# citibeth/spsparse

Hardware: AMD Instinct MI355X
Metric: nnz(C)/s for C=A*A SpGEMM (higher is better)
Workload: dtype f64

## Files before the change

### spsparse_amd/build.py

```python
import os
import subprocess
import sys
from concurrent.futures import ThreadPoolExecutor

HERE = os.path.dirname(os.path.abspath(__file__))
CSRC = os.path.join(HERE, "csrc")
VARIANT = os.environ.get("SPSAMD_VARIANT", "")
LIBDIR = os.path.join(HERE, "lib", VARIANT) if VARIANT else os.path.join(HERE, "lib")
LIB = os.path.join(LIBDIR, "libspsparse_amd.so")
SOURCES = ["prims.hip", "operand.hip", "sink.hip", "consolidate.hip", "spgemm.hip", "symbolic_heavy.hip", "k_light.hip", "k_hash.hip", "k_dense.hip", "k_tiles.hip", "k_spmm.hip", "k_add.hip", "k_stream.hip", "k_masked.hip", "k_sampled.hip", "k_select.hip", "k_extract.hip", "k_reduce.hip", "k_emult.hip",
           "workload.hip", "capi.hip", "dist.hip"]
HEADERS = ["internal.h", "devutil.h", "spgemm_dev.h", "spgemm_host.h", "spgemm_hash.h", "workload_common.h", "x86fp.h", os.path.join("..", "..", "include", "spsparse_amd.h")]
FLAGS = ["--offload-arch=gfx950", "-O3", "-std=c++17", "-fPIC", "-ffp-contract=off",
         "-munsafe-fp-atomics", "-Wall", "-Wno-unused-result"]
FLAGS += os.environ.get("SPSAMD_CXXFLAGS", "").split()


def hipcc():
    for cand in (os.environ.get("HIPCC"), "/opt/rocm/bin/hipcc", "hipcc"):
        if cand and (os.path.isabs(cand) and os.path.exists(cand) or not os.path.isabs(cand)):
            return cand
    return "hipcc"


def _stale(target, deps):
    if not os.path.exists(target):
        return True
    t = os.path.getmtime(target)
    return any(os.path.getmtime(d) > t for d in deps)


def build(force=False, verbose=False):
    os.makedirs(LIBDIR, exist_ok=True)
    hdrs = [os.path.join(CSRC, h) for h in HEADERS]
    objs, jobs = [], []
    for s in SOURCES:
        src = os.path.join(CSRC, s)
        obj = os.path.join(LIBDIR, s.replace(".hip", ".o"))
        objs.append(obj)
        if force or _stale(obj, [src] + hdrs):
            jobs.append([hipcc()] + FLAGS + ["-c", src, "-o", obj])

    def run(cmd):
        if verbose:
            print(" ".join(cmd), flush=True)
        subprocess.check_call(cmd)

    with ThreadPoolExecutor(max_workers=6) as ex:
        list(ex.map(run, jobs))
    if force or jobs or _stale(LIB, objs):
        run([hipcc(), "--offload-arch=gfx950", "-shared", "-fPIC", "-o", LIB] + objs + ["-ldl"])
    return LIB


if __name__ == "__main__":
    print(build(force="--force" in sys.argv, verbose=True))
```

### spsparse_amd/csrc/k_dense.hip

```cpp
#include "spgemm_host.h"

namespace spsamd {


template <int W, int NT, int MODE, bool PAT>
__global__ __launch_bounds__(NT, 4) void k_dense(const Cell *cells, uint32_t ncell, const uint32_t *xb, RowMeta m,
	const uint32_t *widx, uint64_t kstride, uint64_t wstride, uint32_t narrow, EmitParams ep, SinkParams sk, uint32_t *claim_ctr)
{
	constexpr int NW = NT / 64;
	constexpr int NGRP = W / 64;
	constexpr int GPW = NGRP / NW;
	constexpr uint32_t WSHIFT = W == 8192 ? 13 : 14;
	constexpr int R = DENSE_R;
	constexpr int NWORD = W / 64;
	constexpr int WPL = NWORD / 64;
	__shared__ double acc[MODE == MODE_COUNT ? 1 : W + 64];
	__shared__ __attribute__((aligned(16))) uint8_t ctouch[MODE == MODE_COUNT ? W : 16];
	__shared__ uint32_t s_cpref[NT + 1];
	__shared__ uint2 s_cse[NT];
	__shared__ double s_caval[NT];
	__shared__ unsigned long long s_bmask[NWORD];
	__shared__ uint32_t s_scrL[2][NW], s_scrN[2][NW];
	__shared__ uint32_t s_wcnt[NW + 1];
	__shared__ PatCell s_pat;
	__shared__ unsigned long long s_u64[2 * NW];
	__shared__ double s_f64[NW];
	__shared__ uint32_t s_claim[4];

	const unsigned tid = threadIdx.x, lane = lane_id();
	const unsigned wv = (unsigned)__builtin_amdgcn_readfirstlane((int)wave_id());
	const double CLEAN = (PAT && MODE != MODE_COUNT) ? -0.0 : 0.0;
	if (MODE == MODE_COUNT) { for (int q = tid; q < W / 16; q += NT) reinterpret_cast<uint4 *>(ctouch)[q] = make_uint4(0, 0, 0, 0); }
	else for (int q = tid; q < W + 64; q += NT) acc[q] = CLEAN;
	for (int q = tid; q < NWORD; q += NT) s_bmask[q] = 0ull;
	const bool plain = ep.C == 1.0 && !ep.si_pos && !ep.sk_pos;
	const unsigned long long laneK = (unsigned long long)lane * 0x9E3779B97F4A7C15ull;
	unsigned long long d_cnt = 0, d_hash = 0; double d_sum = 0;
	PatAcc pat; pat_init(pat);
	if (tid == 0) pat_reset(&s_pat);
	uint32_t flip = 0;
#ifdef SPSAMD_STAMPS
	unsigned long long st_[12] = {}; unsigned long long st_t = clock64();
#endif

	constexpr uint32_t NONE = 0xFFFFFFFFu;
	const bool claimed = claim_ctr != nullptr && xb != nullptr && !ABL(ep, 16);
	const CellWalk walk = cell_walk(claimed ? nullptr : xb, ncell);
	const uint32_t stride = walk.stride, cend = walk.end;
	const uint32_t clast = ncell ? ncell - 1 : 0;
	uint32_t part = blockIdx.x & 7u, tried = 0;
	auto claim_resolve = [&](uint32_t got) -> uint32_t {
		while (true) {
			if (got < xb[part + 1]) return got;
// ... 66 lines not shown
		STAMP_COUNT(8);
		uint32_t pnseg = 0;
		for (uint32_t chunk = beg; chunk < end; chunk += NT) {
			STAMP_COUNT(9);
			uint32_t lo2, hi2; double a2;
			{
				seg_bounds(kA, w, lo2, hi2);
				a2 = aA;
				if (chunk + NT + tid >= end) hi2 = lo2;
				const uint32_t e2 = chunk + 2 * NT + tid;
				const uint32_t e2c = e2 < end ? e2 : beg;
				kA = m.acol[e2c]; aA = m.aval[e2c];
			}
			const uint32_t items = (len + R - 1) / R;
			const uint32_t inc = wave_inclusive_scan_u32(items);
			const uint64_t nzm = __ballot(len != 0);
			const uint32_t wrank = (uint32_t)__popcll(nzm & lanemask_lt());
			if (lane == 63) s_scrL[flip][wv] = inc;
			if (lane == 0) s_scrN[flip][wv] = (uint32_t)__popcll(nzm);
			STAMP(0);
			lds_barrier();
			STAMP(1);
			if (claimed && chunk == beg) {
				i2 = (uint32_t)__builtin_amdgcn_readfirstlane((int)s_claim[2 + (iter & 1u)]);
				pend2 = cell_pend_load(cells, min(i2, clast), zlane);
			}
			uint32_t baseL = 0, baseN = 0, total = 0, nzc = 0;
#pragma unroll
			for (int q = 0; q < NW; ++q) {
				const uint32_t l = s_scrL[flip][q], n = s_scrN[flip][q];
				if (q < (int)wv) { baseL += l; baseN += n; }
				total += l; nzc += n;
			}
			flip ^= 1u;
			total = (uint32_t)__builtin_amdgcn_readfirstlane((int)total);
			nzc = (uint32_t)__builtin_amdgcn_readfirstlane((int)nzc);
			const uint32_t myfirst = baseL + inc - items;
			if (len) {
				const uint32_t rank = baseN + wrank;
				s_cpref[rank] = myfirst;
				s_cse[rank] = make_uint2(lo, lo + len);
				s_caval[rank] = a;
				if (myfirst < (uint32_t)W) atomicOr(reinterpret_cast<uint32_t *>(s_bmask) + (myfirst >> 5), 1u << (myfirst & 31u));
			}
			if (ABL(ep, 8)) total = 0;
			if (total == 0) { lo = lo2; len = hi2 - lo2; a = a2; continue; }
			if (ep.ordered && MODE != MODE_COUNT) {
				lds_barrier();
				for (uint32_t q = 0; q < nzc; ++q) {
					const uint2 se = s_cse[q];
					const double aq = s_caval[q];
					for (uint32_t t = se.x + tid; t < se.y; t += NT) {
						const BTup bt = m.btup[t];
						const uint32_t slot = (uint32_t)bt.col - wbase;
						acc[slot] = acc[slot] + aq * btup_val(bt);
					}
					lds_barrier();
				}
				for (int q = tid; q < NWORD; q += NT) s_bmask[q] = 0ull;
				lo = lo2; len = hi2 - lo2; a = a2;
				continue;
			}
			uint32_t Q0 = 0;
			for (uint32_t pb = 0; pb < total; pb += W) {
				const uint32_t pe = min(total, pb + (uint32_t)W);
				if (pb) {
					lds_barrier();
					for (int q = tid; q < NWORD; q += NT) s_bmask[q] = 0ull;
					lds_barrier();
					if (len && myfirst >= pb && myfirst < pe) atomicOr(&s_bmask[(myfirst - pb) >> 6], 1ull << ((myfirst - pb) & 63u));
				}
				STAMP(2);
				lds_barrier();
				STAMP(3);
				unsigned long long mw[WPL]; uint32_t pre[WPL];
				uint32_t run = Q0;
#pragma unroll
				for (int x = 0; x < WPL; ++x) {
					mw[x] = s_bmask[x * 64 + lane];
					const uint32_t cnt = (uint32_t)__popcll(mw[x]);
					const uint32_t incl = wave_inclusive_scan_u32(cnt);
					pre[x] = run + incl - cnt;
					run += (uint32_t)__builtin_amdgcn_readlane((int)incl, 63);
				}
				const uint32_t nsteps = (pe - pb + NT - 1) / NT;
				auto lookup = [&](uint32_t step, uint32_t &obp, uint32_t &onv, double &oav) {
					const uint32_t b = step * NW + wv;
					const uint32_t t = pb + (b << 6) + lane;
					const bool ok = t < pe;
					uint32_t mlo = 0, mhi = 0, pr = 0;
#pragma unroll
					for (int x = 0; x < WPL; ++x) {
						if ((b >> 6) == (uint32_t)x) {
							mlo = (uint32_t)__builtin_amdgcn_readlane((int)(uint32_t)mw[x], (int)(b & 63u));
							mhi = (uint32_t)__builtin_amdgcn_readlane((int)(uint32_t)(mw[x] >> 32), (int)(b & 63u));
							pr = (uint32_t)__builtin_amdgcn_readlane((int)pre[x], (int)(b & 63u));
						}
					}
					if (ABL(ep, 128)) { obp = (t * R) & 0xFFFFFu; onv = ok ? R : 0u; oav = 1.0; return; }
					const uint32_t s1lo = (mlo >> 1) | (mhi << 31), s1hi = mhi >> 1;
					const uint32_t qs = pr + (mlo & 1u) - 1u;
					uint32_t q = qs + __builtin_amdgcn_mbcnt_hi(s1hi, __builtin_amdgcn_mbcnt_lo(s1lo, 0u));
					q = min(q, nzc - 1u);
					const uint2 se = s_cse[q];
					obp = se.x + (t - s_cpref[q]) * R;
					onv = ok ? min((uint32_t)R, se.y - obp) : 0u;
					oav = s_caval[q];
				};
				const char *bbase = reinterpret_cast<const char *>(m.btup);
				auto fetch = [&](uint32_t bp_) -> BPiece {
					if (ABL(ep, 64)) bp_ &= 0xFFFFu;
					if (narrow) return *reinterpret_cast<const BPiece *>(bbase + (uint32_t)((bp_ << 3) + (bp_ << 2)));
					return *reinterpret_cast<const BPiece *>(bbase + (uint64_t)bp_ * 12u);
				};
				auto accumulate = [&](const BPiece &piece, uint32_t nv_, double av_) {
#pragma unroll
					for (int u = 0; u < R; ++u) {
						const uint32_t slot = (uint32_t)u < nv_ ? (ABL(ep, 64) ? (piece.w[3 * u] & (W - 1)) : piece.w[3 * u] - wbase) : (uint32_t)W + lane;
						if (ABL(ep, 32)) { if (piece.w[3 * u + 2] == 0x7FF12345u) acc[MODE == MODE_COUNT ? 0 : slot] = av_; }
						else if (MODE == MODE_COUNT) { if ((uint32_t)u < nv_) ctouch[slot] = (uint8_t)1; }
						else {
							const double pv = av_ * __hiloint2double((int)piece.w[3 * u + 2], (int)piece.w[3 * u + 1]);
							atomicAdd(&acc[slot], pv);
							if (PAT && (uint32_t)u < nv_) pat_note(pat, pv);
						}
					}
				};
				STAMP(4);
#if DENSE_DEPTH == 2
				uint32_t bp0, nv0, bp1 = 0, nv1 = 0; double av0, av1 = 0.0;
				lookup(0, bp0, nv0, av0);
				BPiece p0 = fetch(bp0), p1 = p0;
				if (nsteps > 1) lookup(1, bp1, nv1, av1);
				for (uint32_t step = 0; step < nsteps; ++step) {
					STAMP_COUNT(10);
					if (step + 1 < nsteps) p1 = fetch(bp1);
					uint32_t bp2 = 0, nv2 = 0; double av2 = 0.0;
					if (step + 2 < nsteps) lookup(step + 2, bp2, nv2, av2);
					accumulate(p0, nv0, av0);
					p0 = p1; nv0 = nv1; av0 = av1;
					bp1 = bp2; nv1 = nv2; av1 = av2;
				}
#else
				uint32_t bp, nv; double av;
				lookup(0, bp, nv, av);
				for (uint32_t step = 0; step < nsteps; ++step) {
					STAMP_COUNT(10);
					const BPiece piece = fetch(bp);
					uint32_t nbp = bp, nnv = 0; double nav = 0.0;
					if (step + 1 < nsteps) lookup(step + 1, nbp, nnv, nav);
					accumulate(piece, nv, av);
					bp = nbp; nv = nnv; av = nav;
				}
#endif
				Q0 = run;
				STAMP(5);
			}
			if (PAT) { pat_publish(pat, &s_pat); pnseg += nzc; }
			lds_barrier();
			STAMP(6);
			for (int q = tid; q < NWORD; q += NT) s_bmask[q] = 0ull;
			lo = lo2; len = hi2 - lo2; a = a2;
		}
		{
			uint32_t l2, h2;
			seg_bounds(nk, rec1.wa, l2, h2);
			nlo = l2; nlen = nact ? h2 - l2 : 0u;
		}
		if (ABL(ep, 16)) continue;
		STAMP(0);
		uint32_t claim_pending = NONE;
		if (claimed && tid == 0 && tried < 8u) claim_pending = atomicAdd(&claim_ctr[part * 32u], 1u);
		const double pthr = PAT ? pat_threshold(&s_pat, pnseg) : -1.0;
		const uint32_t pbeg = beg, pend = end;
		double v[GPW];
		uint64_t nzmask[GPW];
		uint32_t wcount = 0;
		constexpr unsigned long long MIXK = 0x9E3779B97F4A7C15ull;
		unsigned long long X0 = ((((unsigned long long)(uint32_t)rowid) << 32) | (unsigned long long)(wbase + wv * GPW * 64u)) * MIXK;
		X0 = ((unsigned long long)(uint32_t)__builtin_amdgcn_readfirstlane((int)(uint32_t)(X0 >> 32)) << 32) |
			(unsigned long long)(uint32_t)__builtin_amdgcn_readfirstlane((int)(uint32_t)X0);
		double r_sum = 0;
		unsigned long long r_hash = 0;
		if constexpr (MODE == MODE_COUNT) {
			static_assert(W / 16 == NT, "sixteen flag bytes per thread");
			uint32_t cnt = 0;
			{
				uint4 *cw = reinterpret_cast<uint4 *>(ctouch);
				const uint4 x = cw[tid];
				const uint32_t xs[4] = {x.x, x.y, x.z, x.w};
				if (x.x | x.y | x.z | x.w) {
					cw[tid] = make_uint4(0, 0, 0, 0);
#pragma unroll
					for (int q = 0; q < 4; ++q) {
						if (!ep.sk_pos) cnt += (uint32_t)__popc(xs[q]);
						else {
#pragma unroll
							for (int b = 0; b < 4; ++b)
								if (((xs[q] >> (8 * b)) & 1u) && col_allowed(ep, (int32_t)(wbase + tid * 16u + (uint32_t)(4 * q + b)))) ++cnt;
						}
					}
				}
			}
			wcount = (uint32_t)wave_reduce_sum((unsigned long long)cnt);
		} else {
#pragma unroll
		for (int gi = 0; gi < GPW; ++gi) {
			int grp = wv * GPW + gi;
			double x = acc[grp * 64 + lane];
			acc[grp * 64 + lane] = CLEAN;
			bool ok;
			if (MODE != MODE_COUNT && PAT) {
				const bool touched = __double_as_longlong(x) != (long long)0x8000000000000000ull;
				x = pat_fix_wave(touched && !(fabs(x) > pthr), x, (int32_t)(wbase + grp * 64 + lane), m, pbeg, pend);
			}
			if (plain) ok = x != 0;
			else ok = emit_value(ep, a_scale, (int32_t)(wbase + grp * 64 + lane), x, &x);
			v[gi] = x;
			nzmask[gi] = __ballot(ok);
			wcount += (uint32_t)__popcll(nzmask[gi]);
			if (MODE == MODE_DIGEST) {
				unsigned long long h = X0 + laneK;
				h ^= h >> 29;
				r_hash += ok ? h : 0ull;
				if (plain && !PAT) r_sum += x;
				else r_sum += ok ? x : 0.0;
				X0 += 64ull * MIXK;
			}
		}
		}
		if (MODE == MODE_DIGEST) {
			if (lane == 0) d_cnt += wcount;
			d_sum += r_sum;
			d_hash += r_hash;
			if (sk.row_nnz) {
				double rs = wave_reduce_sum(r_sum);
				r_hash = wave_reduce_sum(r_hash);
				if (lane == 0 && wcount) { atomicAdd((unsigned long long *)&sk.row_nnz[rowid], (unsigned long long)wcount); atomicAdd(&sk.row_sum[rowid], rs); atomicAdd(&sk.row_hash[rowid], r_hash); }
			}
		} else {
			if (lane == 0) s_wcnt[wv] = wcount;
			__syncthreads();
			uint32_t wbefore = 0, wtotal = 0;
#pragma unroll
			for (int q = 0; q < NW; ++q) { uint32_t t = s_wcnt[q]; if (q < (int)wv) wbefore += t; wtotal += t; }
			if (MODE == MODE_COUNT) {
				if (tid == 0) sk.segcount[cell.seg] = wtotal;
			} else {
				int64_t o = sk.segoff[cell.seg] + wbefore;
#pragma unroll
				for (int gi = 0; gi < GPW; ++gi) {
					uint64_t mk = nzmask[gi];
					if ((mk >> lane) & 1ull) {
						int64_t oo = o + __popcll(mk & lanemask_lt());
						sk.out_i[oo] = rowid;
						sk.out_j[oo] = (int32_t)(wbase + (wv * GPW + gi) * 64 + lane);
						sk.out_v[oo] = v[gi];
					}
					o += __popcll(mk);
				}
				if (tid == 0) sk.segactual[cell.seg] = wtotal;
			}
			__syncthreads();
// ... 69 lines not shown
```

### spsparse_amd/csrc/k_tiles.hip

```cpp
#include "spgemm_host.h"
#include "spgemm_hash.h"

namespace spsamd {

constexpr uint32_t TILE_NONE = 0xFFFFFFFFu;


template <int MODE, bool PAT>
__global__ __launch_bounds__(TILE2_NT, 4) void k_hash_tiles2(const Tile *tiles, uint32_t ntile, const TCell *tcells, RowMeta m,
	const uint32_t *bwin, uint32_t nwin1, uint32_t narrow, EmitParams ep, SinkParams sk, uint32_t *claim_ctr)
{
	constexpr int NT = TILE2_NT, T = TILE2_T, NW = NT / 64, R = DENSE_R;
	constexpr int NWORD = TILE2_ITEMS / 64;
	constexpr int MAXST = 3;
	__shared__ int32_t h_key[T + 64];
	__shared__ double h_val[MODE == MODE_COUNT ? 1 : T];
	__shared__ uint16_t occ[T / 2];
	__shared__ uint64_t s_sort[MODE == MODE_STORE ? T / 2 : 1];
	__shared__ uint16_t s_cnt[MODE == MODE_STORE ? 16 * ((T / 2 + NT - 1) / NT) * (NT / 64) : 1];
	__shared__ TileX<NT, NWORD> X;
	__shared__ uint32_t scr32[NW + 1];
	__shared__ uint32_t s_nocc;
	__shared__ PatCell s_pat;
	__shared__ unsigned long long s_u64[2 * NW];
	__shared__ double s_f64[NW];
	__shared__ uint32_t s_claim[4];

	const unsigned tid = threadIdx.x, lane = lane_id();
	const unsigned wv = (unsigned)__builtin_amdgcn_readfirstlane((int)wave_id());
	for (int q = tid; q < T; q += NT) { h_key[q] = -1; if (MODE != MODE_COUNT) h_val[q] = 0.0; }
	if (tid < 64) h_key[T + tid] = -1;
	for (int q = tid; q < NWORD; q += NT) X.bmask[q] = 0ull;
	if (tid == 0) s_nocc = 0;
	PatAcc pat; pat_init(pat);
	if (tid == 0) pat_reset(&s_pat);
	DigestAcc dacc{0, 0, 0.0};
	uint32_t flip = 0;
	const char *bbase = reinterpret_cast<const char *>(m.btup);
#ifdef SPSAMD_STAMPS
	unsigned long long st_[12] = {}; unsigned long long st_t = clock64();
#endif

	const bool claimed = claim_ctr != nullptr;
	const uint32_t stride = gridDim.x;
	const uint32_t tlast = ntile - 1;
	uint32_t i0, i1;
	if (claimed) {
		if (tid == 0) for (int q = 0; q < 3; ++q) { const uint32_t got = atomicAdd(claim_ctr, 1u); s_claim[q == 2 ? 3 : q] = got < ntile ? got : TILE_NONE; }
		__syncthreads();
		i0 = s_claim[0]; i1 = s_claim[1];
	} else {
		i0 = blockIdx.x;
		i1 = i0 + stride < ntile ? i0 + stride : TILE_NONE;
	}
// ... 100 lines not shown
							const double pv = av * __hiloint2double((int)piece.w[3 * u + 2], (int)piece.w[3 * u + 1]);
							atomicAdd(&h_val[h[u]], pv);
							if (PAT) pat_note(pat, pv);
						}
					}
					newmask[u] = __ballot(isnew[u]);
					nnew += (uint32_t)__popcll(newmask[u]);
				}
				if (nnew) {
					uint32_t base = 0;
					if (lane == 0) base = lds_add_rtn_u32(&s_nocc, nnew);
					base = (uint32_t)__builtin_amdgcn_readfirstlane((int)base);
#pragma unroll
					for (int u = 0; u < R; ++u) {
						if (isnew[u]) occ[base + __popcll(newmask[u] & lanemask_lt())] = (uint16_t)h[u];
						base += (uint32_t)__popcll(newmask[u]);
					}
				}
			}
			if (PAT) pat_publish(pat, &s_pat);
			STAMP(3);
			lds_barrier();
			STAMP(4);
			const uint32_t nocc = s_nocc;
			if (c + 1 < tile.ncells) {
				tile_lookup(X, tab, nzc, (i1 >> 6) + wv, X.cellI[c + 2], pbp, pnv, pav);
				ppiece = fetch_piece(bbase, pbp, narrow);
			}
			uint32_t colbase = 0, colbits = 0;
			if (MODE == MODE_STORE) {
				const uint32_t wab = X.cellw[c];
				const uint32_t wa = wab & 0xFFFFu, wb = wab >> 16;
				colbase = wa << ep.wshift;
				colbits = ep.wshift + (wb - wa > 1 ? 32 - __builtin_clz(wb - wa - 1u) : 0);
			}
			STAMP(5);
			const double pthr = PAT ? pat_threshold(&s_pat, tile.end - tile.beg) : -1.0;
			hash_emit<T, NT, MODE, PAT>(nocc, rowid, seg, ep, sk, h_key, h_val, occ, s_sort, scr32, dacc, s_cnt, colbase, colbits, m, tile.beg, tile.end, pthr);
			if (PAT) { lds_barrier(); if (tid == 0) pat_reset(&s_pat); }
			if (tid == 0) s_nocc = 0;
			STAMP(6);
			lds_barrier();
			STAMP(7);
		}
		for (int q = tid; q < NWORD; q += NT) X.bmask[q] = 0ull;
	}
#ifdef SPSAMD_STAMPS
	if (tid == 0 && sk.stamps) for (int i = 0; i < 12; ++i) sk.stamps[(size_t)blockIdx.x * 12 + i] = st_[i];
#endif
	if (MODE == MODE_DIGEST) digest_flush<NT>(sk.digest, dacc.cnt, dacc.hash, dacc.sum, s_u64, s_f64);
}


template <int MODE, bool PAT>
__global__ __launch_bounds__(BM_NT, 4) void k_bm_tiles(const Tile *tiles, uint32_t ntile, const TCell *tcells, RowMeta m,
	const uint32_t *bwin, uint32_t nwin1, uint32_t narrow, EmitParams ep, SinkParams sk, uint32_t *claim_ctr)
{
	constexpr int NT = BM_NT, NW = NT / 64, R = DENSE_R;
	constexpr int NWORD = BM_ITEMS / 64;
	constexpr int MAXST = (BM_MAXOUT / R + (int)TILE_LMAX + 64 + NT - 1) / NT;
	constexpr int WPT = BM_WORDS / NT;
	__shared__ __attribute__((aligned(16))) unsigned long long bm[BM_WORDS];
	__shared__ __attribute__((aligned(8))) uint16_t bpre[BM_WORDS];
	__shared__ double acc[BM_MAXOUT];
	__shared__ uint32_t colof[BM_MAXOUT];
	__shared__ TileX<NT, NWORD> X;
	__shared__ uint32_t s_wtot[2][NW];
	__shared__ uint32_t s_wbase[NW];
	__shared__ PatCell s_pat;
	__shared__ uint32_t s_scan[NW + 1];
	__shared__ unsigned long long s_u64[2 * NW];
	__shared__ double s_f64[NW];
	__shared__ uint32_t s_claim[4];

	const unsigned tid = threadIdx.x, lane = lane_id();
	const unsigned wv = (unsigned)__builtin_amdgcn_readfirstlane((int)wave_id());
	for (int q = tid; q < BM_WORDS; q += NT) bm[q] = 0ull;
	for (int q = tid; q < BM_MAXOUT; q += NT) acc[q] = 0.0;
	for (int q = tid; q < NWORD; q += NT) X.bmask[q] = 0ull;
	const bool plain = ep.C == 1.0 && !ep.si_pos && !ep.sk_pos;
	unsigned long long d_cnt = 0, d_hash = 0; double d_sum = 0;
	PatAcc pat; pat_init(pat);
	if (PAT && tid == 0) pat_reset(&s_pat);
	uint32_t flip = 0, sflip = 0;
	const char *bbase = reinterpret_cast<const char *>(m.btup);
#ifdef SPSAMD_STAMPS
	unsigned long long st_[12] = {}; unsigned long long st_t = clock64();
#endif

	const bool claimed = claim_ctr != nullptr;
	const uint32_t stride = gridDim.x;
	const uint32_t tlast = ntile - 1;
	uint32_t i0, i1;
	if (claimed) {
		if (tid == 0) for (int q = 0; q < 3; ++q) { const uint32_t got = atomicAdd(claim_ctr, 1u); s_claim[q == 2 ? 3 : q] = got < ntile ? got : TILE_NONE; }
		__syncthreads();
		i0 = s_claim[0]; i1 = s_claim[1];
	} else {
		i0 = blockIdx.x;
		i1 = i0 + stride < ntile ? i0 + stride : TILE_NONE;
	}
	i0 = (uint32_t)__builtin_amdgcn_readfirstlane((int)i0); i1 = (uint32_t)__builtin_amdgcn_readfirstlane((int)i1);
	Tile rec1 = tiles[min(i0, tlast)];
	uint32_t nlo, nlen, nseg_, nw_; double na;
	{
		const uint32_t L = rec1.end - rec1.beg;
		uint32_t lsh = 0;
		while ((1u << lsh) < L) ++lsh;
		const uint32_t c = tid >> lsh, ei = tid & ((1u << lsh) - 1u);
		const bool act = c < rec1.ncells && ei < L;
		const uint32_t ec = rec1.beg + (ei < L ? ei : 0u);
		const TCell tc = tcells[rec1.first + (c < rec1.ncells ? c : 0u)];
		const uint32_t *bw = bwin + (uint64_t)(uint32_t)m.acol[ec] * nwin1;
		const uint32_t lo = bw[tc.wa], hi = bw[tc.wb];
// ... 36 lines not shown
		{
			const uint32_t *bw = bwin + (uint64_t)(uint32_t)nk * nwin1;
			const uint32_t nlo_ = bw[ntc.wa], nhi_ = bw[ntc.wb];
			nlo = nlo_; nlen = nact ? nhi_ - nlo_ : 0u; nseg_ = ntc.seg; nw_ = (uint32_t)ntc.wa | ((uint32_t)ntc.wb << 16);
		}
		if (total == 0 || nzc == 0) {
			if (MODE != MODE_DIGEST) for (uint32_t c = tid; c < tile.ncells; c += NT) { if (MODE == MODE_COUNT) sk.segcount[X.cellseg[c]] = 0; else sk.segactual[X.cellseg[c]] = 0; }
			continue;
		}
		TileTab<NWORD / 64> tab;
		tile_tables(X, tab);

		uint32_t pbp, pnv; double pav;
		tile_lookup(X, tab, nzc, (X.cellI[0] >> 6) + wv, X.cellI[1], pbp, pnv, pav);
		BPiece ppiece = fetch_piece(bbase, pbp, narrow);
#ifndef BM_D2
#define BM_D2 1
#endif
		constexpr bool D2 = BM_D2 && MODE != MODE_STORE;
		uint32_t qnv = 0; double qav = 0; BPiece qpiece;
		if (D2 && ((X.cellI[1] - X.cellI[0]) >> 6) > (uint32_t)NW + wv) {
			uint32_t qbp;
			tile_lookup(X, tab, nzc, (X.cellI[0] >> 6) + NW + wv, X.cellI[1], qbp, qnv, qav);
			qpiece = fetch_piece(bbase, qbp, narrow);
		}
		STAMP(0);
		for (uint32_t c = 0; c < tile.ncells; ++c) {
			STAMP_COUNT(11);
			const uint32_t i0 = X.cellI[c], i1 = X.cellI[c + 1];
			const uint32_t seg = X.cellseg[c];
			const uint32_t nblk = (i1 - i0) >> 6;
			const uint32_t wab = X.cellw[c];
			const uint32_t colbase = (wab & 0xFFFFu) << ep.wshift;
			const uint32_t nwords = ((wab >> 16) - (wab & 0xFFFFu)) << (ep.wshift - 6);
			if ((nblk > (uint32_t)(MAXST * NW) || nwords > (uint32_t)BM_WORDS) && tid == 0) atomicOr(sk.err, 2u);
			uint32_t krel[MAXST][R]; double kval[MODE == MODE_COUNT ? 1 : MAXST][MODE == MODE_COUNT ? 1 : R];
#pragma unroll
			for (int st = 0; st < MAXST; ++st) {
#pragma unroll
				for (int u = 0; u < R; ++u) krel[st][u] = 0xFFFFFFFFu;
				const uint32_t bl = (uint32_t)st * NW + wv;
				if (st > 0 && bl >= nblk) continue;
				uint32_t nv; double av; BPiece piece;
				if (st == 0) { nv = bl < nblk ? pnv : 0u; av = pav; piece = ppiece; }
				else if (D2 && st == 1) { nv = qnv; av = qav; piece = qpiece; }
				else {
					uint32_t bp;
					tile_lookup(X, tab, nzc, (i0 >> 6) + bl, i1, bp, nv, av);
					piece = fetch_piece(bbase, bp, narrow);
				}
#pragma unroll
				for (int u = 0; u < R; ++u) {
					if ((uint32_t)u < nv) {
						const uint32_t rel = piece.w[3 * u] - colbase;
						krel[st][u] = rel;
						if constexpr (MODE != MODE_COUNT) {
							kval[st][u] = av * __hiloint2double((int)piece.w[3 * u + 2], (int)piece.w[3 * u + 1]);
							if (PAT) pat_note(pat, kval[st][u]);
						}
						atomicOr(reinterpret_cast<uint32_t *>(bm) + (rel >> 5), 1u << (rel & 31u));
					}
				}
			}
			if (PAT && MODE != MODE_COUNT) pat_publish(pat, &s_pat);
			STAMP(2);
			lds_barrier();
			STAMP(3);
			const double pthr = (PAT && MODE != MODE_COUNT) ? pat_threshold(&s_pat, tile.end - tile.beg) : -1.0;
			uint32_t wcnt[WPT], mine = 0;
			{
				unsigned long long wd[WPT];
#pragma unroll
				for (int x = 0; x < WPT; ++x) wd[x] = bm[tid * WPT + x];
				if (c + 1 < tile.ncells) {
					const uint32_t i2 = X.cellI[c + 2];
					tile_lookup(X, tab, nzc, (i1 >> 6) + wv, i2, pbp, pnv, pav);
					ppiece = fetch_piece(bbase, pbp, narrow);
					if (D2 && ((i2 - i1) >> 6) > (uint32_t)NW + wv) {
						uint32_t qbp;
						tile_lookup(X, tab, nzc, (i1 >> 6) + NW + wv, i2, qbp, qnv, qav);
						qpiece = fetch_piece(bbase, qbp, narrow);
					}
				}
#pragma unroll
				for (int x = 0; x < WPT; ++x) { wcnt[x] = (uint32_t)__popcll(wd[x]); mine += wcnt[x]; }
			}
			const uint32_t inc = wave_inclusive_scan_u32(mine);
			if (lane == 63) s_wtot[sflip][wv] = inc;
			{
				static_assert(WPT == 4, "packed prefix store");
				const uint32_t r0 = inc - mine, r1 = r0 + wcnt[0], r2 = r1 + wcnt[1], r3 = r2 + wcnt[2];
				reinterpret_cast<uint2 *>(bpre)[tid] = make_uint2(r0 | (r1 << 16), r2 | (r3 << 16));
			}
			STAMP(4);
			lds_barrier();
			STAMP(5);
			if (PAT && MODE != MODE_COUNT && tid == 0) pat_reset(&s_pat);
			uint32_t distinct;
			{
				const uint32_t t = lane < (unsigned)NW ? s_wtot[sflip][lane] : 0u;
				const uint32_t ti = wave_inclusive_scan_u32(t);
				if (lane < (unsigned)NW) s_wbase[lane] = ti - t;
				distinct = (uint32_t)__builtin_amdgcn_readlane((int)ti, NW - 1);
			}
			sflip ^= 1u;
			if (MODE == MODE_COUNT && !ep.sk_pos) {
				if (tid == 0) sk.segcount[seg] = distinct;
#pragma unroll
				for (int x = 0; x < WPT; ++x) { const uint32_t w = tid * WPT + x; if (w < nwords && wcnt[x]) bm[w] = 0ull; }
				lds_barrier();
				continue;
			}
			STAMP(4);
			if constexpr (MODE != MODE_COUNT) {
#pragma unroll
				for (int st = 0; st < MAXST; ++st) {
					if ((uint32_t)st * NW + wv >= nblk) continue;
					uint32_t pre[R], wb[R]; unsigned long long wd[R];
#pragma unroll
					for (int u = 0; u < R; ++u) {
						const uint32_t w = (krel[st][u] >> 6) & (uint32_t)(BM_WORDS - 1);
						pre[u] = bpre[w]; wb[u] = s_wbase[w / (64 * WPT)]; wd[u] = bm[w];
					}
#pragma unroll
					for (int u = 0; u < R; ++u) {
						const uint32_t rel = krel[st][u];
						if (rel != 0xFFFFFFFFu) {
							const uint32_t rank = wb[u] + pre[u] + (uint32_t)__popcll(wd[u] & ((1ull << (rel & 63u)) - 1ull));
							atomicAdd(&acc[rank], kval[st][u]);
							colof[rank] = rel;
						}
					}
				}
				STAMP(6);
				lds_barrier();
				STAMP(7);
			}
			if constexpr (MODE != MODE_COUNT) {
				if (mine) { uint4 *z = reinterpret_cast<uint4 *>(&bm[tid * WPT]); z[0] = make_uint4(0, 0, 0, 0); z[1] = make_uint4(0, 0, 0, 0); }
			}
			if constexpr (MODE == MODE_DIGEST) {
				unsigned long long cnt = 0, rh = 0; double vs = 0;
				auto note = [&](uint32_t rel, double v) {
					const int32_t col = (int32_t)(colbase + rel);
					const bool ok = plain ? v != 0 : emit_value(ep, a_scale, col, v, &v);
					if (ok) { ++cnt; rh += mix64((uint32_t)rowid, (uint32_t)col); vs += v; }
				};
				if constexpr (!PAT) {
					unsigned long long *acc64 = reinterpret_cast<unsigned long long *>(acc);
					for (uint32_t i = tid; i < distinct; i += 2 * NT) {
						const uint32_t j = i + NT;
						const bool two = j < distinct;
						const uint32_t jj = two ? j : i;
						const uint32_t rel0 = colof[i], rel1 = colof[jj];
						const double v0 = __longlong_as_double((long long)atomicExch(&acc64[i], 0ull));
						const double v1 = __longlong_as_double((long long)atomicExch(&acc64[jj], 0ull));
						note(rel0, v0);
						if (two) note(rel1, v1);
					}
				} else {
					for (uint32_t base = 0; base < distinct; base += NT) {
						const uint32_t i = base + tid;
						const bool valid = i < distinct;
						const uint32_t rel = valid ? colof[i] : 0u;
						double v = valid ? acc[i] : 0.0;
						if (valid) acc[i] = 0.0;
						v = pat_fix_wave(valid && !(fabs(v) > pthr), v, (int32_t)(colbase + rel), m, tile.beg, tile.end);
						if (valid) note(rel, v);
					}
				}
				d_cnt += cnt; d_sum += vs; d_hash += rh;
				if (sk.row_nnz) {
					const unsigned long long rc = wave_reduce_sum(cnt); const double rs = wave_reduce_sum(vs);
					rh = wave_reduce_sum(rh);
					if (lane == 0 && rc) { atomicAdd((unsigned long long *)&sk.row_nnz[rowid], rc); atomicAdd(&sk.row_sum[rowid], rs); atomicAdd(&sk.row_hash[rowid], rh); }
				}
			} else if constexpr (MODE == MODE_COUNT) {
				uint32_t cnt = 0;
#pragma unroll
				for (int x = 0; x < WPT; ++x) {
					if (!wcnt[x]) continue;
					const uint32_t w = tid * WPT + x;
					unsigned long long word = bm[w];
					bm[w] = 0ull;
					while (word) {
						const uint32_t bit = (uint32_t)__builtin_ctzll(word);
						word &= word - 1ull;
						if (col_allowed(ep, (int32_t)(colbase + (w << 6) + bit))) ++cnt;
					}
				}
				uint32_t tot;
				block_exclusive_scan<uint32_t, NT>(cnt, s_scan, &tot);
				if (tid == 0) sk.segcount[seg] = tot;
			} else {
				const int64_t o = sk.segoff[seg];
				uint32_t nbad = 0, run = 0;
				int any_bad;
				if (!ep.sk_pos) {
					for (uint32_t base = 0; base < distinct; base += NT) {
						const uint32_t i = base + tid;
						const bool valid = i < distinct;
						const uint32_t rel = valid ? colof[i] : 0u;
						double v = 1.0;
						if (valid) { v = acc[i]; acc[i] = 0.0; }
						if (PAT) v = pat_fix_wave(valid && !(fabs(v) > pthr), v, (int32_t)(colbase + rel), m, tile.beg, tile.end);
						const bool ok = !valid || (plain ? v != 0 : emit_value(ep, a_scale, (int32_t)(colbase + rel), v, &v));
						if (valid) { sk.out_i[o + i] = rowid; sk.out_j[o + i] = ok ? (int32_t)(colbase + rel) : -1; sk.out_v[o + i] = v; }
						if (!ok) ++nbad;
					}
					any_bad = __syncthreads_or((int)nbad);
					if (any_bad) {
						for (uint32_t ibase = 0; ibase < distinct; ibase += NT) {
							const uint32_t i = ibase + tid;
							int32_t col = -1; double v = 0;
							if (i < distinct) { col = sk.out_j[o + i]; v = sk.out_v[o + i]; }
							const bool ok = col >= 0;
							uint32_t tot;
// ... 218 lines not shown
				lds_barrier();
				if (tid == 0) { sk.segcount[seg] = s_count; s_count = 0; }
				lds_barrier();
			} else {
				lds_barrier();
				if (wv == 0) {
					uint32_t run = 0;
#pragma unroll
					for (int x = 0; x < NWORD / 64; ++x) {
						const uint32_t cnt = (uint32_t)__popcll(s_cbm[x * 64 + lane]);
						const uint32_t inc2 = wave_inclusive_scan_u32(cnt);
						s_cpre[x * 64 + lane] = run + inc2 - cnt;
						run += (uint32_t)__builtin_amdgcn_readlane((int)inc2, 63);
					}
					if (lane == 0) s_cpre[NWORD] = run;
				}
				lds_barrier();
				const int64_t o = sk.segoff[seg];
#pragma unroll
				for (int st = 0; st < MAXST; ++st) {
#pragma unroll
					for (int u = 0; u < R; ++u) {
						const uint32_t slot = ks[st][u];
						if (slot < (uint32_t)W) {
							const uint32_t wd = slot >> 6;
							const uint32_t rank = s_cpre[wd] + (uint32_t)__popcll(s_cbm[wd] & ((1ull << (slot & 63u)) - 1ull));
							sk.out_i[o + rank] = rowid;
							sk.out_j[o + rank] = (int32_t)(wbase + slot);
							sk.out_v[o + rank] = kv[st][u];
						}
					}
				}
				if (tid == 0) sk.segactual[seg] = s_cpre[NWORD];
				lds_barrier();
				for (int q = tid; q < NWORD; q += NT) s_cbm[q] = 0ull;
				lds_barrier();
			}
		}
		for (int q = tid; q < NWORD; q += NT) X.bmask[q] = 0ull;
	}
	if (MODE == MODE_DIGEST) digest_flush<NT>(sk.digest, d_cnt, d_hash, d_sum, s_u64, s_f64);
}

template <int MODE>
void launch_tiles_bm(spsamd_ctx *c, const Heavy &hv, const RowMeta &m, const EmitParams &ep, const SinkParams &sk)
{
	const uint32_t narrow = ((uint64_t)hv.nnzb + DENSE_R) * 12u < (uint64_t(1) << 32) ? 1u : 0u;
	const unsigned grid = std::min<unsigned>(hv.ntile, (unsigned)c->num_cu * 2u);
	uint32_t *claim = hv.tile_ctr ? hv.tile_ctr + (MODE == MODE_STORE ? 1 : 0) : nullptr;
#ifdef SPSAMD_STAMPS
	SinkParams sk2 = sk;
	sk2.stamps = c->arena.get<unsigned long long>((size_t)grid * 12);
	fill_zero(c, sk2.stamps, (size_t)grid * 12 * sizeof(unsigned long long));
	k_bm_tiles<MODE, false><<<dim3(grid), dim3(BM_NT), 0, c->stream>>>(hv.tb.tiles, hv.ntile, hv.tb.tcells, m, hv.bwin, hv.nwin1, narrow, ep, sk2, claim);
	{
		std::vector<unsigned long long> h((size_t)grid * 12);
		SPS_HIP(hipMemcpyAsync(h.data(), sk2.stamps, h.size() * 8, hipMemcpyDeviceToHost, c->stream));
		SPS_HIP(hipStreamSynchronize(c->stream));
		double sum[12] = {};
		for (unsigned g = 0; g < grid; ++g) for (int i = 0; i < 12; ++i) sum[i] += (double)h[(size_t)g * 12 + i];
		static const char *nm[12] = {"pre", "expand", "bits", "B", "scan", "B", "rank-add", "B", "emit", "B", "tiles", "cells"};
		fprintf(stderr, "k_bm_tiles stamps (mean cycles per workgroup, grid %u):", grid);
		for (int i = 0; i < 12; ++i) fprintf(stderr, " %s %.4g", nm[i], sum[i] / grid);
		fprintf(stderr, "\n");
	}
#else
	if (ep.pattern) k_bm_tiles<MODE, true><<<dim3(grid), dim3(BM_NT), 0, c->stream>>>(hv.tb.tiles, hv.ntile, hv.tb.tcells, m, hv.bwin, hv.nwin1, narrow, ep, sk, claim);
	else k_bm_tiles<MODE, false><<<dim3(grid), dim3(BM_NT), 0, c->stream>>>(hv.tb.tiles, hv.ntile, hv.tb.tcells, m, hv.bwin, hv.nwin1, narrow, ep, sk, claim);
#endif
	SPS_LAUNCH_CHECK();
}

template <int MODE>
void launch_tiles_hash2(spsamd_ctx *c, const Heavy &hv, const RowMeta &m, const EmitParams &ep, const SinkParams &sk)
{
	const uint32_t narrow = ((uint64_t)hv.nnzb + DENSE_R) * 12u < (uint64_t(1) << 32) ? 1u : 0u;
	static int per_cu2 = 0;
	if (!per_cu2) {
		int nb = 0;
		if (hipOccupancyMaxActiveBlocksPerMultiprocessor(&nb, k_hash_tiles2<MODE, false>, TILE2_NT, 0) != hipSuccess || nb < 1) nb = 1;
		per_cu2 = nb;
	}
	const unsigned grid = std::min<unsigned>(hv.ntile, (unsigned)(c->num_cu * per_cu2));
	uint32_t *claim = hv.tile_ctr ? hv.tile_ctr + (MODE == MODE_STORE ? 1 : 0) : nullptr;
#ifdef SPSAMD_STAMPS
	SinkParams sk2 = sk;
	sk2.stamps = c->arena.get<unsigned long long>((size_t)grid * 12);
	fill_zero(c, sk2.stamps, (size_t)grid * 12 * sizeof(unsigned long long));
	k_hash_tiles2<MODE, false><<<dim3(grid), dim3(TILE2_NT), 0, c->stream>>>(hv.tb.tiles, hv.ntile, hv.tb.tcells, m, hv.bwin, hv.nwin1, narrow, ep, sk2, claim);
	{
		std::vector<unsigned long long> h((size_t)grid * 12);
		SPS_HIP(hipMemcpyAsync(h.data(), sk2.stamps, h.size() * 8, hipMemcpyDeviceToHost, c->stream));
		SPS_HIP(hipStreamSynchronize(c->stream));
		double sum[12] = {};
		for (unsigned g = 0; g < grid; ++g) for (int i = 0; i < 12; ++i) sum[i] += (double)h[(size_t)g * 12 + i];
		static const char *nm[12] = {"pre", "expand", "tables+pf", "insert", "Bwait", "pf-next", "emit", "Bwait2", "tiles", "cells", "-", "-"};
		fprintf(stderr, "k_hash_tiles2 stamps (mean cycles per workgroup, grid %u):", grid);
		for (int i = 0; i < 10; ++i) fprintf(stderr, " %s %.4g", nm[i], sum[i] / grid);
		fprintf(stderr, "\n");
	}
#else
	if (ep.pattern) k_hash_tiles2<MODE, true><<<dim3(grid), dim3(TILE2_NT), 0, c->stream>>>(hv.tb.tiles, hv.ntile, hv.tb.tcells, m, hv.bwin, hv.nwin1, narrow, ep, sk, claim);
	else k_hash_tiles2<MODE, false><<<dim3(grid), dim3(TILE2_NT), 0, c->stream>>>(hv.tb.tiles, hv.ntile, hv.tb.tcells, m, hv.bwin, hv.nwin1, narrow, ep, sk, claim);
#endif
	SPS_LAUNCH_CHECK();
}

template <int MODE>
void launch_tiles_direct(spsamd_ctx *c, const Heavy &hv, const RowMeta &m, const EmitParams &ep, const SinkParams &sk)
{
	RowMeta m2 = m;
	m2.btup = hv.btw;
	const uint32_t narrow = ((uint64_t)hv.nnzb + DENSE_R) * 12u < (uint64_t(1) << 32) ? 1u : 0u;
	if (hv.W == 8192) {
		const unsigned grid = std::min<unsigned>(hv.ntile2, (unsigned)c->num_cu * 2u);
		k_direct_tiles<8192, 512, MODE><<<dim3(grid), dim3(512), 0, c->stream>>>(hv.tb2.tiles, hv.ntile2, hv.tb2.tcells, m2, hv.wptr, hv.nrowb, narrow, ep, sk);
	} else {
		const unsigned grid = std::min<unsigned>(hv.ntile2, (unsigned)c->num_cu);
		k_direct_tiles<16384, 1024, MODE><<<dim3(grid), dim3(1024), 0, c->stream>>>(hv.tb2.tiles, hv.ntile2, hv.tb2.tcells, m2, hv.wptr, hv.nrowb, narrow, ep, sk);
	}
	SPS_LAUNCH_CHECK();
// ... 14 lines not shown
```

Measured before the change: 143.9 billion.

## Swizzle dense accumulator slots and hash tile bitmap keys to spread LDS banks

Adds an XOR swizzle to the dense-window accumulator so each 64-slot group is permuted by a per-group constant. The intent is to spread atomicAdd traffic from clustered columns across LDS banks. Separately, the bitmap-tiles kernel now maps relative columns through an invertible multiplicative key for digest and non-positional count modes, again to scatter bitmap and accumulator accesses. Keys are inverted at emit time, which costs extra ALU work per entry, and this path breaks column-ordered ranks, so it is disabled for store mode.

```diff
diff --git a/spsparse_amd/build.py b/spsparse_amd/build.py
--- a/spsparse_amd/build.py
+++ b/spsparse_amd/build.py
@@ -10,7 +10,7 @@
 LIB = os.path.join(LIBDIR, "libspsparse_amd.so")
 SOURCES = ["prims.hip", "operand.hip", "sink.hip", "consolidate.hip", "spgemm.hip", "symbolic_heavy.hip", "k_light.hip", "k_hash.hip", "k_dense.hip", "k_tiles.hip", "k_spmm.hip", "k_add.hip", "k_stream.hip", "k_masked.hip", "k_sampled.hip", "k_select.hip", "k_extract.hip", "k_reduce.hip", "k_emult.hip",
            "workload.hip", "capi.hip", "dist.hip"]
-HEADERS = ["internal.h", "devutil.h", "spgemm_dev.h", "spgemm_host.h", "spgemm_hash.h", "workload_common.h", "x86fp.h", os.path.join("..", "..", "include", "spsparse_amd.h")]
+HEADERS = ["internal.h", "devutil.h", "bank_layout.h", "spgemm_dev.h", "spgemm_host.h", "spgemm_hash.h", "workload_common.h", "x86fp.h", os.path.join("..", "..", "include", "spsparse_amd.h")]
 FLAGS = ["--offload-arch=gfx950", "-O3", "-std=c++17", "-fPIC", "-ffp-contract=off",
          "-munsafe-fp-atomics", "-Wall", "-Wno-unused-result"]
 FLAGS += os.environ.get("SPSAMD_CXXFLAGS", "").split()
diff --git a/spsparse_amd/csrc/bank_layout.h b/spsparse_amd/csrc/bank_layout.h
--- /dev/null
+++ b/spsparse_amd/csrc/bank_layout.h
@@ -0,0 +1,26 @@
+#pragma once
+#include <stdint.h>
+#include "workload_common.h"
+
+namespace spsamd {
+
+SPS_HD uint32_t dense_swz(uint32_t group) { return ((group * 181u) >> 3) & 63u; }
+SPS_HD uint32_t dense_phys(uint32_t slot) { return slot ^ dense_swz(slot >> 6); }
+
+constexpr uint32_t TILE_KEY_BITS = 17, TILE_KEY_MASK = (1u << TILE_KEY_BITS) - 1u;
+constexpr uint32_t TILE_KEY_LOW_BITS = 14, TILE_KEY_LOW = (1u << TILE_KEY_LOW_BITS) - 1u;
+constexpr uint32_t TILE_KEY_K = 40503u, TILE_KEY_KINV = 96135u;
+static_assert(((TILE_KEY_K * TILE_KEY_KINV) & TILE_KEY_MASK) == 1u, "inverse modulo 2^17, hence modulo 2^14");
+
+SPS_HD uint32_t bank_mul24(uint32_t x, uint32_t k)
+{
+#if defined(__HIP_DEVICE_COMPILE__)
+	return __umul24(x, k);
+#else
+	return x * k;
+#endif
+}
+SPS_HD uint32_t tile_key(uint32_t rel) { return rel ^ ((rel ^ bank_mul24(rel, TILE_KEY_K)) & TILE_KEY_LOW); }
+SPS_HD uint32_t tile_rel(uint32_t key) { return key ^ ((key ^ bank_mul24(key, TILE_KEY_KINV)) & TILE_KEY_LOW); }
+
+}
diff --git a/spsparse_amd/csrc/k_dense.hip b/spsparse_amd/csrc/k_dense.hip
--- a/spsparse_amd/csrc/k_dense.hip
+++ b/spsparse_amd/csrc/k_dense.hip
@@ -1,4 +1,5 @@
 #include "spgemm_host.h"
+#include "bank_layout.h"
 
 namespace spsamd {
 
@@ -171,7 +172,7 @@
 					const double aq = s_caval[q];
 					for (uint32_t t = se.x + tid; t < se.y; t += NT) {
 						const BTup bt = m.btup[t];
-						const uint32_t slot = (uint32_t)bt.col - wbase;
+						const uint32_t slot = dense_phys((uint32_t)bt.col - wbase);
 						acc[slot] = acc[slot] + aq * btup_val(bt);
 					}
 					lds_barrier();
@@ -235,7 +236,8 @@
 				auto accumulate = [&](const BPiece &piece, uint32_t nv_, double av_) {
 #pragma unroll
 					for (int u = 0; u < R; ++u) {
-						const uint32_t slot = (uint32_t)u < nv_ ? (ABL(ep, 64) ? (piece.w[3 * u] & (W - 1)) : piece.w[3 * u] - wbase) : (uint32_t)W + lane;
+						const uint32_t col = ABL(ep, 64) ? (piece.w[3 * u] & (W - 1)) : piece.w[3 * u] - wbase;
+						const uint32_t slot = (uint32_t)u < nv_ ? (MODE == MODE_COUNT ? col : dense_phys(col)) : (uint32_t)W + lane;
 						if (ABL(ep, 32)) { if (piece.w[3 * u + 2] == 0x7FF12345u) acc[MODE == MODE_COUNT ? 0 : slot] = av_; }
 						else if (MODE == MODE_COUNT) { if ((uint32_t)u < nv_) ctouch[slot] = (uint8_t)1; }
 						else {
@@ -326,8 +328,9 @@
 #pragma unroll
 		for (int gi = 0; gi < GPW; ++gi) {
 			int grp = wv * GPW + gi;
-			double x = acc[grp * 64 + lane];
-			acc[grp * 64 + lane] = CLEAN;
+			const uint32_t ps = grp * 64 + (lane ^ (uint32_t)__builtin_amdgcn_readfirstlane((int)dense_swz((uint32_t)grp)));
+			double x = acc[ps];
+			acc[ps] = CLEAN;
 			bool ok;
 			if (MODE != MODE_COUNT && PAT) {
 				const bool touched = __double_as_longlong(x) != (long long)0x8000000000000000ull;
diff --git a/spsparse_amd/csrc/k_tiles.hip b/spsparse_amd/csrc/k_tiles.hip
--- a/spsparse_amd/csrc/k_tiles.hip
+++ b/spsparse_amd/csrc/k_tiles.hip
@@ -1,5 +1,7 @@
 #include "spgemm_host.h"
 #include "spgemm_hash.h"
+#include "bank_layout.h"
+#include <type_traits>
 
 namespace spsamd {
 
@@ -206,7 +208,7 @@
 }
 
 
-template <int MODE, bool PAT>
+template <int MODE, bool PAT, bool KEY>
 __global__ __launch_bounds__(BM_NT, 4) void k_bm_tiles(const Tile *tiles, uint32_t ntile, const TCell *tcells, RowMeta m,
 	const uint32_t *bwin, uint32_t nwin1, uint32_t narrow, EmitParams ep, SinkParams sk, uint32_t *claim_ctr)
 {
@@ -214,6 +216,9 @@
 	constexpr int NWORD = BM_ITEMS / 64;
 	constexpr int MAXST = (BM_MAXOUT / R + (int)TILE_LMAX + 64 + NT - 1) / NT;
 	constexpr int WPT = BM_WORDS / NT;
+	static_assert(!KEY || MODE != MODE_STORE, "the COO store wants rank order to be column order");
+	static_assert(!KEY || BM_WORDS * 64 == (1 << TILE_KEY_BITS), "the keys fill the bitmap");
+	static_assert(!KEY || (BM_WORDS / NW) * 64 == (1 << TILE_KEY_LOW_BITS), "a key stays in the words of its column's wave");
 	__shared__ __attribute__((aligned(16))) unsigned long long bm[BM_WORDS];
 	__shared__ __attribute__((aligned(8))) uint16_t bpre[BM_WORDS];
 	__shared__ double acc[BM_MAXOUT];
@@ -356,7 +361,7 @@
 #pragma unroll
 				for (int u = 0; u < R; ++u) {
 					if ((uint32_t)u < nv) {
-						const uint32_t rel = piece.w[3 * u] - colbase;
+						const uint32_t rel = KEY ? tile_key(piece.w[3 * u] - colbase) : piece.w[3 * u] - colbase;
 						krel[st][u] = rel;
 						if constexpr (MODE != MODE_COUNT) {
 							kval[st][u] = av * __hiloint2double((int)piece.w[3 * u + 2], (int)piece.w[3 * u + 1]);
@@ -411,7 +416,7 @@
 			if (MODE == MODE_COUNT && !ep.sk_pos) {
 				if (tid == 0) sk.segcount[seg] = distinct;
 #pragma unroll
-				for (int x = 0; x < WPT; ++x) { const uint32_t w = tid * WPT + x; if (w < nwords && wcnt[x]) bm[w] = 0ull; }
+				for (int x = 0; x < WPT; ++x) { const uint32_t w = tid * WPT + x; if ((KEY || w < nwords) && wcnt[x]) bm[w] = 0ull; }
 				lds_barrier();
 				continue;
 			}
@@ -459,14 +464,14 @@
 						const uint32_t rel0 = colof[i], rel1 = colof[jj];
 						const double v0 = __longlong_as_double((long long)atomicExch(&acc64[i], 0ull));
 						const double v1 = __longlong_as_double((long long)atomicExch(&acc64[jj], 0ull));
-						note(rel0, v0);
-						if (two) note(rel1, v1);
+						note(KEY ? tile_rel(rel0) : rel0, v0);
+						if (two) note(KEY ? tile_rel(rel1) : rel1, v1);
 					}
 				} else {
 					for (uint32_t base = 0; base < distinct; base += NT) {
 						const uint32_t i = base + tid;
 						const bool valid = i < distinct;
-						const uint32_t rel = valid ? colof[i] : 0u;
+						const uint32_t rel = valid ? (KEY ? tile_rel(colof[i]) : colof[i]) : 0u;
 						double v = valid ? acc[i] : 0.0;
 						if (valid) acc[i] = 0.0;
 						v = pat_fix_wave(valid && !(fabs(v) > pthr), v, (int32_t)(colbase + rel), m, tile.beg, tile.end);
@@ -791,7 +796,7 @@
 	SinkParams sk2 = sk;
 	sk2.stamps = c->arena.get<unsigned long long>((size_t)grid * 12);
 	fill_zero(c, sk2.stamps, (size_t)grid * 12 * sizeof(unsigned long long));
-	k_bm_tiles<MODE, false><<<dim3(grid), dim3(BM_NT), 0, c->stream>>>(hv.tb.tiles, hv.ntile, hv.tb.tcells, m, hv.bwin, hv.nwin1, narrow, ep, sk2, claim);
+	k_bm_tiles<MODE, false, MODE == MODE_DIGEST><<<dim3(grid), dim3(BM_NT), 0, c->stream>>>(hv.tb.tiles, hv.ntile, hv.tb.tcells, m, hv.bwin, hv.nwin1, narrow, ep, sk2, claim);
 	{
 		std::vector<unsigned long long> h((size_t)grid * 12);
 		SPS_HIP(hipMemcpyAsync(h.data(), sk2.stamps, h.size() * 8, hipMemcpyDeviceToHost, c->stream));
@@ -804,8 +809,13 @@
 		fprintf(stderr, "\n");
 	}
 #else
-	if (ep.pattern) k_bm_tiles<MODE, true><<<dim3(grid), dim3(BM_NT), 0, c->stream>>>(hv.tb.tiles, hv.ntile, hv.tb.tcells, m, hv.bwin, hv.nwin1, narrow, ep, sk, claim);
-	else k_bm_tiles<MODE, false><<<dim3(grid), dim3(BM_NT), 0, c->stream>>>(hv.tb.tiles, hv.ntile, hv.tb.tcells, m, hv.bwin, hv.nwin1, narrow, ep, sk, claim);
+	auto go = [&](auto pat, auto key) {
+		k_bm_tiles<MODE, decltype(pat)::value, decltype(key)::value><<<dim3(grid), dim3(BM_NT), 0, c->stream>>>(hv.tb.tiles, hv.ntile, hv.tb.tcells, m, hv.bwin, hv.nwin1, narrow, ep, sk, claim);
+	};
+	auto go_pat = [&](auto key) { if (ep.pattern) go(std::true_type{}, key); else go(std::false_type{}, key); };
+	if constexpr (MODE == MODE_DIGEST) go_pat(std::true_type{});
+	else if constexpr (MODE == MODE_COUNT) { if (ep.sk_pos) go_pat(std::false_type{}); else go_pat(std::true_type{}); }
+	else go_pat(std::false_type{});
 #endif
 	SPS_LAUNCH_CHECK();
 }
```

Result: faster. 150.3 billion, median of 6 (+4.4%).
